# jasonyaw/CDAE

Hardware: AMD Instinct MI355X
Metric: users/sec (whole node) K=200 ML-10M-shape; Recall@10 parity (higher is better)
Workload: dtype f32

## Files before the change

cdae_amd/csrc/cdae_hip.hip:

```cpp
#include <hip/hip_runtime.h>

#include <cstring>

#include <rocprim/rocprim.hpp>

#include <algorithm>
#include <atomic>
#include <condition_variable>
#include <deque>
#include <mutex>
#include <thread>
#include <chrono>
#include <cmath>
#include <cstdarg>
#include <cstdlib>
#include <cstdio>
#include <cstring>
#include <numeric>
#include <string>
#include <vector>

#include "../../include/cdae_hip.h"
#include "cdae_internal.hpp"
#include "cdae_kernels.hpp"
// ... 61 lines not shown
  uint32_t K = 0, Kp = 0, NI = 1, B = 0;
  uint64_t uid_offset = 0;
  cdae::HyperParams hp{};

  std::vector<int64_t> h_row_ptr;
  int64_t* d_row_ptr = nullptr;
  uint32_t* d_col = nullptr;
  uint32_t* d_item_order = nullptr;
  uint32_t hot_rows = 0;
  uint32_t late_rows = 0;
  float* d_Ghot = nullptr;
  uint32_t* d_hotdup = nullptr;
  uint32_t* d_late_bits = nullptr;
  uint32_t late_words = 0;
  bool fused_decode = false;
  bool fused_possible = false;
  bool allow_fused = true;
  uint32_t* h_err = nullptr;
  int err_slot = -1;
  uint32_t* d_fused_err = nullptr;
  cdae::FusedGeom fused_geo{};
  bool fused_geo_set = false;
  std::vector<float> h_rank_len;
  uint32_t* d_cold_map = nullptr;
  uint32_t num_cus = 256;
  cdae::DecodeLate decode_late() const { return cdae::DecodeLate{d_Ghot, d_hotdup, late_rows}; }
  cdae::LateFinish late_finish() { return cdae::LateFinish{d_Ghot, d_hotdup, d_item_order, d_D0, d_dup_corr, late_rows}; }
  bool full_unfused = false;
  std::vector<uint32_t> h_unit_ptr;
  uint32_t* d_rank_of = nullptr;
  uint32_t* d_unit_user = nullptr;
  uint32_t* d_unit_ptr = nullptr;
  uint32_t unit_cap = 0;
  float* d_Hpart = nullptr;
  uint32_t* d_uptr_tmp = nullptr;

  float* d_shared = nullptr;
  size_t n_shared = 0, n_matrix = 0;
  size_t off[CDAE_P_COUNT] = {0};
  size_t cnt[CDAE_P_COUNT] = {0};
  float* d_Wu = nullptr;
  float* d_Wu_ag = nullptr;
  float* d_Uu = nullptr;
  float* d_Uu_ag = nullptr;
  float* d_Ssum = nullptr;
  float* d_delta_rows = nullptr;

  uint64_t Ecap = 0;
  struct ExBuf {
    uint32_t* item = nullptr; uint64_t* val = nullptr;
    uint32_t* sorted_item = nullptr; uint64_t* sorted_val = nullptr;
    uint32_t* seg = nullptr;
    uint16_t* key16 = nullptr; uint16_t* sorted_key16 = nullptr;
    uint32_t* dup_of_pos = nullptr; uint32_t* dup_of_ex = nullptr;
    uint32_t* dup_count = nullptr;
    uint32_t* item_count = nullptr; uint32_t* prefix = nullptr; uint32_t* rank = nullptr; uint64_t* bucketed = nullptr;
    uint32_t* tile_hist = nullptr; uint32_t* block_total = nullptr;
    uint32_t* wg_state = nullptr;
    uint32_t* cells = nullptr; uint32_t* cell_flag = nullptr;
    uint32_t cell_tag = 0;
    hipEvent_t ready = nullptr, released = nullptr;
  } ex[3];
  static constexpr int NSETS = 3;
  hipStream_t prep2 = nullptr;
  bool prep2_own = false;
  bool prep2_auto = false;
  float* d_D0 = nullptr;
  uint32_t dup_stripes = 1;
  float* d_dup_corr = nullptr; uint32_t dup_cap = 0;
  float* d_HGpart = nullptr;
  uint32_t Bp = 0, Ip = 0;
  __bf16 *d_Zb = nullptr, *d_ZTb = nullptr, *d_Db = nullptr, *d_DTb = nullptr, *d_Gb = nullptr, *d_GTb = nullptr;
  float* d_dD = nullptr;
  uint8_t* d_has_in = nullptr;
  uint32_t* d_iota = nullptr;
  uint32_t* d_bits_train = nullptr;
  size_t bits_stride = 0;
  uint32_t full_slices = 1;
  bool db_valid = false;
  bool db_rows_valid = false;
  uint32_t zb_rows = 0xFFFFFFFFu;
  uint32_t full_one_stream_max = 2048;
  hipStream_t aux = nullptr;
// ... 195 lines not shown
    float t = 0.f;
    HIPCHK(hipEventElapsedTime(&t, s.a, s.b));
    ms[s.family] += t;
    launches[s.family]++;
    h->pool.push_back(s.a); h->pool.push_back(s.b);
  }
  h->spans.clear();
  if (st) {
    st->ms_sample = ms[F_SAMPLE]; st->ms_sort = ms[F_SORT]; st->ms_encode = ms[F_ENCODE];
    st->ms_decode = ms[F_DECODE]; st->ms_hidden = ms[F_HIDDEN]; st->ms_input = ms[F_INPUT];
    st->launches_decode = launches[F_DECODE];
  }
  return 0;
}

template <class F, class... P> int visit_slots(F& f, P*&... p) {
  int rc = 0;
  ((rc = rc ? rc : f((void**)&p)), ...);
  return rc;
}
template <class F> int visit_device_ptrs(cdae_hip* h, F f) {
  for (auto& b : h->ex)
    CHK(visit_slots(f, b.item, b.val, b.sorted_item, b.sorted_val, b.seg, b.dup_of_pos, b.dup_of_ex, b.dup_count, b.key16, b.sorted_key16,
                    b.item_count, b.prefix, b.rank, b.bucketed, b.tile_hist, b.block_total, b.wg_state, b.cells, b.cell_flag));
  return visit_slots(f, h->d_row_ptr, h->d_col, h->d_item_order, h->d_shared, h->d_Wu, h->d_Wu_ag, h->d_D0, h->d_HGpart, h->d_sort_tmp,
                     h->d_unit_ptr, h->d_Hpart, h->d_uptr_tmp, h->d_Zb, h->d_ZTb, h->d_Db, h->d_DTb, h->d_Gb, h->d_GTb, h->d_dD, h->d_has_in,
                     h->d_Z, h->d_Dz, h->d_HG, h->d_G, h->d_touched, h->d_uids, h->d_rec, h->d_base, h->d_delta, h->d_recv, h->d_snap,
                     h->d_dup_corr, h->d_unit_user, h->d_zeval, h->d_bits, h->d_hpart_eval, h->d_iota, h->d_bits_train,
                     h->d_Uu, h->d_Uu_ag, h->d_Ssum, h->d_delta_rows, h->d_score, h->d_Hsum, h->d_hsum_eval, h->d_iota_eval, h->d_rec_score,
                     h->d_gpos, h->d_ub, h->d_ub_ag, h->d_UVpre, h->d_rank_of, h->d_grow_ptr, h->d_gcol, h->d_gunit_ptr, h->d_gunit_user,
                     h->d_test_ptr, h->d_test_col, h->d_topn_pu, h->d_topn_out, h->d_bucket_cut, h->d_range_of,
                     h->d_Ghot, h->d_hotdup, h->d_late_bits, h->d_cold_map,
                     h->d_rows_ptr, h->d_rows_uid, h->d_rows_col, h->d_rows_tptr, h->d_rows_pu, h->d_rows_tcol, h->d_rows_out);
}

void free_all(cdae_hip* h) {
  (void)visit_device_ptrs(h, [](void** p) { if (*p) (void)hipFree(*p); *p = nullptr; return 0; });
  if (h->d_scalar) (void)hipFree(h->d_scalar);
  for (auto& b : h->ex) {
    if (b.ready) (void)hipEventDestroy(b.ready);
    if (b.released) (void)hipEventDestroy(b.released);
  }
  if (h->h_err) { err_slot_release(h->device, h->err_slot); h->h_err = nullptr; h->d_fused_err = nullptr; h->err_slot = -1; }
  if (h->prep) (void)hipStreamDestroy(h->prep);
  if (h->prep2 && h->prep2_own) (void)hipStreamDestroy(h->prep2);
  if (h->aux) (void)hipStreamDestroy(h->aux);
  if (h->ev_fork) (void)hipEventDestroy(h->ev_fork);
// ... 75 lines not shown
                       use_cells ? x.cells : (uint32_t*)nullptr, x.cell_flag, x.cell_tag);
  } else
  hipLaunchKernelGGL(sample_kernel, dim3((n_units + 3) / 4), dim3(256), 0, st, h->hp, h->d_row_ptr, h->d_col,
                     h->d_unit_ptr + bt.s0, n_units, bt.s0, bt.nb, bt.cidx, seed, epoch, x.item, x.val, x.key16,
                     x.seg, h->counting_sort || bucket ? 0u : 4u * I, x.dup_count, x.dup_of_ex, h->d_unit_user,
                     x.wg_state, (const uint32_t*)h->d_gpos, 0u, 0u, 0u,
                     (const uint16_t*)(use_cells ? h->d_range_of : nullptr), (const uint32_t*)h->d_bucket_cut, h->bucket_ranges,
                     use_cells ? x.cells : (uint32_t*)nullptr, x.cell_flag, x.cell_tag);
  CHK(pr.end());
  CHK(pr.begin(h, F_SORT, st, prof_q));
  const dim3 seg_grid((uint32_t)((bt.E + 256 * SEG_PER_THREAD - 1) / (256 * SEG_PER_THREAD)));
  if (bt.E == 0) {
  } else if (h->mf_seq && !h->prep_force_sort) {
  } else if (bucket) {
    if (!h->bucket_attr_set) {
      HIPCHK(hipFuncSetAttribute((const void*)bucket_sort_kernel, hipFuncAttributeMaxDynamicSharedMemorySize, (int)BK_LDS_BYTES));
      h->bucket_attr_set = true;
    }
    hipLaunchKernelGGL(bucket_sort_kernel, dim3(h->bucket_ranges), dim3(BK_THREADS), BK_LDS_BYTES, st, (const uint16_t*)x.key16, (const uint64_t*)x.val,
                       (uint32_t)bt.E, (const uint32_t*)h->d_bucket_cut, x.wg_state, (const uint32_t*)(use_cells ? x.cells : nullptr), n_units,
                       (const uint32_t*)x.cell_flag, x.cell_tag, x.seg, x.seg + I, (const uint32_t*)h->d_rank_of,
                       x.seg + 2 * (size_t)I, x.seg + 3 * (size_t)I, x.sorted_val, x.bucketed, x.dup_count, h->dup_cap, x.dup_of_pos, x.dup_of_ex,
                       h->dup_stripes, h->d_fused_err);
  } else if (h->counting_sort) {
    const uint32_t n_tiles = (uint32_t)((bt.E + TILE_EX - 1) / TILE_EX);
    const size_t tile_lds = (size_t)I * sizeof(uint32_t);
    if (tile_lds + 1024 > 64 * 1024 && !h->tile_attr_set) {
      HIPCHK(hipFuncSetAttribute((const void*)tile_hist_kernel, hipFuncAttributeMaxDynamicSharedMemorySize, (int)tile_lds));
      HIPCHK(hipFuncSetAttribute((const void*)tile_scatter_kernel, hipFuncAttributeMaxDynamicSharedMemorySize, (int)tile_lds + 1024));
      h->tile_attr_set = true;
    }
    hipLaunchKernelGGL(tile_hist_kernel, dim3(n_tiles), dim3(TILE_THREADS), tile_lds / 2 + 4, st, x.item, (uint32_t)bt.E, I, x.tile_hist);
    hipLaunchKernelGGL(item_tile_scan_kernel, dim3((I + 255) / 256), dim3(256), 0, st, x.tile_hist, n_tiles, I, x.item_count, x.rank, x.block_total);
    hipLaunchKernelGGL(tile_scatter_kernel, dim3(n_tiles), dim3(TILE_THREADS), tile_lds + 128 * sizeof(uint32_t), st, x.item, x.val,
                       (uint32_t)bt.E, I, x.tile_hist, x.item_count, x.rank, x.block_total, x.prefix, x.seg, x.seg + I, x.dup_count, x.bucketed,
                       (const uint32_t*)h->d_rank_of, x.seg + 2 * (size_t)I, x.seg + 3 * (size_t)I);
    hipLaunchKernelGGL(segment_sort_kernel, dim3((I + SEGSORT_ITEMS - 1) / SEGSORT_ITEMS), dim3(SEGSORT_THREADS), 0, st, I, x.prefix, x.bucketed,
                       x.sorted_val, x.item_count, x.dup_count, h->dup_cap, x.dup_of_pos, x.dup_of_ex, h->dup_stripes);
  } else if (x.key16) {
    HIPCHK(rocprim::radix_sort_pairs(sort_tmp, h->sort_tmp_bytes, x.key16, x.sorted_key16, x.val, x.sorted_val,
                                     (size_t)bt.E, 0u, (unsigned)h->sort_bits, st));
    hipLaunchKernelGGL(segment_kernel<uint16_t>, seg_grid, dim3(256), 0, st, x.sorted_key16, x.sorted_val, (uint32_t)bt.E,
                       x.seg, x.seg + I, x.dup_count, h->dup_cap, x.dup_of_pos, x.dup_of_ex, h->dup_stripes,
                       (const uint32_t*)h->d_rank_of, x.seg + 2 * (size_t)I, x.seg + 3 * (size_t)I, shs ? I : 0xFFFFFFFFu);
  } else {
    HIPCHK(rocprim::radix_sort_pairs(sort_tmp, h->sort_tmp_bytes, x.item, x.sorted_item, x.val, x.sorted_val,
                                     (size_t)bt.E, 0u, (unsigned)h->sort_bits, st));
    hipLaunchKernelGGL(segment_kernel<uint32_t>, seg_grid, dim3(256), 0, st, x.sorted_item, x.sorted_val, (uint32_t)bt.E,
                       x.seg, x.seg + I, x.dup_count, h->dup_cap, x.dup_of_pos, x.dup_of_ex, h->dup_stripes,
                       (const uint32_t*)h->d_rank_of, x.seg + 2 * (size_t)I, x.seg + 3 * (size_t)I, shs ? I : 0xFFFFFFFFu);
  }
  CHK(pr.end());
  if (h->cfg.full_output && h->d_bits_train) {
    const uint32_t words = (I + 31) / 32;
    uint32_t* bits = h->d_bits_train + (size_t)b * h->bits_stride;
    hipLaunchKernelGGL(rated_bits_kernel, dim3((bt.nb + 3) / 4), dim3(256), 0, st, h->d_row_ptr, h->d_col, bt.s0, bt.nb, words, bits);
  }
  HIPCHK(hipEventRecord(x.ready, st));
  HIPCHK(hipGetLastError());
  return 0;
}

int fused_geometry(cdae_hip* h, uint32_t hot, uint32_t I) {
  using namespace cdae;
  FusedGeom g{};
  g.hot_wgs = (hot + 3) / 4;
  const uint32_t n_groups = (I - hot + 3) / 4, S = h->num_cus;
  std::vector<float> len(n_groups, 0.f);
  for (uint32_t q = 0; q < n_groups; ++q)
    for (uint32_t j = 0; j < 4 && hot + 4 * q + j < I; ++j) len[q] = std::max(len[q], h->h_rank_len[hot + 4 * q + j]);
  std::vector<uint32_t> by_len(n_groups);
  std::iota(by_len.begin(), by_len.end(), 0u);
  std::stable_sort(by_len.begin(), by_len.end(), [&](uint32_t a, uint32_t b2) { return len[a] > len[b2]; });
  const uint32_t cu0 = std::min(g.hot_wgs, S > 8 ? S - 8 : 0u);
  const uint32_t n_bins = (S - cu0) * 4;
  std::vector<std::vector<uint32_t>> bin(n_bins);
  {
    using Ent = std::pair<float, uint32_t>;
    std::vector<Ent> heap;
    for (uint32_t i = 0; i < n_bins; ++i) heap.push_back({0.f, i});
    auto cmp = [](const Ent& a, const Ent& b2) { return a.first > b2.first || (a.first == b2.first && a.second > b2.second); };
    std::make_heap(heap.begin(), heap.end(), cmp);
    for (uint32_t k = 0; k < n_groups; ++k) {
      const uint32_t q = by_len[k];
      std::pop_heap(heap.begin(), heap.end(), cmp);
      Ent e = heap.back();
      bin[e.second].push_back(q);
      e.first += 4.f + len[q];
      heap.back() = e;
      std::push_heap(heap.begin(), heap.end(), cmp);
    }
  }
  size_t rounds_cold = 0;
  for (auto& v : bin) rounds_cold = std::max(rounds_cold, v.size());
  g.decode_wgs = (uint32_t)std::max<size_t>(rounds_cold, 1) * S;
  std::vector<uint32_t> map((size_t)g.decode_wgs * 4, 0xFFFFFFFFu);
  for (uint32_t i = 0; i < n_bins; ++i) {
    const uint32_t cu = cu0 + i / 4, w = i % 4;
    for (size_t k = 0; k < bin[i].size(); ++k) map[((size_t)k * S + cu) * 4 + w] = bin[i][k];
  }
  if (h->d_cold_map) { HIPCHK(hipFree(h->d_cold_map)); h->d_cold_map = nullptr; }
  CHK(dev_alloc(&h->d_cold_map, map.size()));
  HIPCHK(hipMemcpy(h->d_cold_map, map.data(), map.size() * sizeof(uint32_t), hipMemcpyHostToDevice));
  g.cold_map = h->d_cold_map;
  h->fused_geo = g;
  h->fused_geo_set = true;
  return 0;
}

int launch_decode(cdae_hip* h, cdae_hip::ExBuf& x, const cdae::GatherArgs* fused = nullptr) {
  using namespace cdae;
  hipStream_t st = h->stream;
  const uint32_t I = (uint32_t)h->I;
  const dim3 blk(256);
  const dim3 grid_rows((I + 3) / 4);
#define DECODE_TAIL h->d_item_order, x.seg + 2 * (size_t)I, x.seg + 3 * (size_t)I, x.sorted_val, h->d_Z, h->dec(), h->dec_ag(), \
                    h->P(CDAE_P_BP), h->P(CDAE_P_BP_AG), h->d_HG, h->d_G, h->d_D0, h->d_touched, x.dup_of_pos, h->d_dup_corr
#define DECODE_ARGS h->hp, DECODE_TAIL
#define DECODE_LA(NI_, L_, A_)                                                                                       \
  do {                                                                                                               \
    if (pad) hipLaunchKernelGGL((decode_rows_kernel<NI_, L_, A_, true>), grid_rows, blk, 0, st, DECODE_ARGS);        \
    else hipLaunchKernelGGL((decode_rows_kernel<NI_, L_, A_, false>), grid_rows, blk, 0, st, DECODE_ARGS);           \
  } while (0)
#define DECODE_NI(NI_)                                          \
  do {                                                          \
    if (ce && ada) DECODE_LA(NI_, 5, true);                     \
    else if (ce) DECODE_LA(NI_, 5, false);                      \
    else if (ada) DECODE_LA(NI_, 0, true);                      \
    else DECODE_LA(NI_, 0, false);                              \
  } while (0)
#define DECODE_HY(NV_, NT_)                                                                                           \
  do {                                                                                                                \
    if (fused) {                                                                                                       \
      if (ce && ada) hipLaunchKernelGGL((decode_gather_kernel<NV_, NT_, 5, true>), grid_fu, blk, 0, st, h->hp, hot, geo, late, *fused, DECODE_TAIL);   \
      else if (ce) hipLaunchKernelGGL((decode_gather_kernel<NV_, NT_, 5, false>), grid_fu, blk, 0, st, h->hp, hot, geo, late, *fused, DECODE_TAIL);    \
      else if (ada) hipLaunchKernelGGL((decode_gather_kernel<NV_, NT_, 0, true>), grid_fu, blk, 0, st, h->hp, hot, geo, late, *fused, DECODE_TAIL);    \
      else hipLaunchKernelGGL((decode_gather_kernel<NV_, NT_, 0, false>), grid_fu, blk, 0, st, h->hp, hot, geo, late, *fused, DECODE_TAIL);            \
    }                                                                                                                  \
    else if (ce && ada) hipLaunchKernelGGL((decode_hybrid_kernel<NV_, NT_, 5, true>), grid_hy, blk, 0, st, h->hp, hot, late, DECODE_TAIL);   \
    else if (ce) hipLaunchKernelGGL((decode_hybrid_kernel<NV_, NT_, 5, false>), grid_hy, blk, 0, st, h->hp, hot, late, DECODE_TAIL);    \
    else if (ada) hipLaunchKernelGGL((decode_hybrid_kernel<NV_, NT_, 0, true>), grid_hy, blk, 0, st, h->hp, hot, late, DECODE_TAIL);    \
    else hipLaunchKernelGGL((decode_hybrid_kernel<NV_, NT_, 0, false>), grid_hy, blk, 0, st, h->hp, hot, late, DECODE_TAIL);            \
  } while (0)
#define DECODE_HY_NT(NV_)                                                                        \
  do {                                                                                           \
    if (nt == 1) DECODE_HY(NV_, 1); else if (nt == 2) DECODE_HY(NV_, 2); else DECODE_HY(NV_, 4); \
  } while (0)
  {
    const bool ce = h->cfg.loss_type == CDAE_LOSS_CROSS_ENTROPY, ada = h->cfg.using_adagrad != 0, pad = h->K < h->Kp;
    const uint32_t K = h->K;
    if (K <= 256) {
      const uint32_t hot = std::min<uint32_t>(h->hot_rows, I);
      const uint32_t waves = hot + (I - hot + 3) / 4;
      const dim3 grid_hy((waves + 3) / 4);
      const DecodeLate late = h->decode_late();
      if (fused && !h->fused_geo_set) CHK(fused_geometry(h, hot, I));
      const FusedGeom geo = h->fused_geo;
      const dim3 grid_fu(geo.decode_wgs + (fused ? 8u * ((fused->n_units + 3u) / 4u) : 0u));
      const uint32_t nv = K / 64, tail = K % 64;
      const uint32_t nt = tail == 0 ? 0u : (tail < 16 ? 1u : (tail < 32 ? 2u : 4u));
      if (nt == 0) {
        switch (nv) { case 1: DECODE_HY(1, 0); break; case 2: DECODE_HY(2, 0); break; case 3: DECODE_HY(3, 0); break; default: DECODE_HY(4, 0); break; }
      } else {
        switch (nv) { case 0: DECODE_HY_NT(0); break; case 1: DECODE_HY_NT(1); break; case 2: DECODE_HY_NT(2); break; default: DECODE_HY_NT(3); break; }
      }
    } else {
      switch (h->NI) { case 1: DECODE_NI(1); break; case 2: DECODE_NI(2); break; case 4: DECODE_NI(4); break; default: DECODE_NI(8); break; }
    }
  }
#undef DECODE_HY_NT
#undef DECODE_HY
#undef DECODE_LA
#undef DECODE_NI
#undef DECODE_ARGS
#undef DECODE_TAIL
  HIPCHK(hipGetLastError());
  return 0;
}
// ... 37 lines not shown
  float* const ghot = h->late_rows ? h->d_Ghot : nullptr;
  uint32_t* const gfill = fused ? reinterpret_cast<uint32_t*>(h->d_G) : nullptr;
  const uint32_t n_fill = fused ? (uint32_t)bt.E : 0u;
  if (!explicit_in && !h->encode_two_launches && nb <= ENCODE_USERS_MAX) {
    DISPATCH_NI(h->NI, encode_users_kernel, dim3(nb), dim3(ENC_WAVES * WAVE), 0, st, h->hp, h->d_row_ptr, h->d_col, h->P(CDAE_P_W), uptr, s0, nb,
                bt.cidx, seed, epoch, h->d_Wu, h->P(CDAE_P_B), h->d_Z, h->d_Dz, h->d_HG, h->d_Uu, h->d_Ssum,
                (BF16_T*)nullptr, (BF16_T*)nullptr, 0u, (float*)nullptr, (const float*)nullptr, (const float*)nullptr, (const uint32_t*)nullptr,
                ghot, h->d_hotdup, gfill, n_fill);
  } else {
    DISPATCH_NI(h->NI, encode_partial_kernel, grid_units, blk, 0, st, h->hp, h->d_row_ptr, h->d_col, h->P(CDAE_P_W), uptr, n_units,
                (const uint32_t*)nullptr, s0, nb, 1, CDAE_STREAM_CORRUPT, bt.cidx, seed, epoch, h->d_Hpart, explicit_in, n_explicit,
                explicit_in ? (const uint32_t*)nullptr : (const uint32_t*)h->d_unit_user);
    DISPATCH_NI(h->NI, encode_finish_kernel, grid_users, blk, 0, st, h->hp, h->d_Hpart, uptr, h->d_Wu, h->P(CDAE_P_B),
                (const uint32_t*)nullptr, s0, nb, 1, h->d_Z, h->d_Dz, h->d_HG, h->d_Uu, h->d_Ssum,
                (BF16_T*)nullptr, (BF16_T*)nullptr, 0u, ghot, h->d_hotdup, gfill, n_fill);
  }
  CHK(pr.end());

  if (!h->skip_ready_wait) HIPCHK(hipStreamWaitEvent(st, x.ready, 0));
  const GatherArgs ga{h->d_row_ptr, uptr, n_units, s0, nb, x.item, h->d_G, h->d_D0, h->d_HGpart, explicit_in ? (uint32_t)bt.E : 0u, x.dup_of_ex,
                      h->d_dup_corr, explicit_in ? (const uint32_t*)nullptr : (const uint32_t*)h->d_unit_user,
                      h->late_rows ? (const uint32_t*)h->d_late_bits : (const uint32_t*)nullptr, h->late_words, h->d_fused_err};
  CHK(pr.begin(h, F_DECODE, st));
  CHK(launch_decode(h, x, fused ? &ga : nullptr));
  CHK(pr.end());

  CHK(pr.begin(h, F_HIDDEN, st));
  if (!fused)
    DISPATCH_NI(h->NI, hidden_gather_kernel, dim3(8 * ((n_units + 3) / 4)), blk, 0, st, h->hp, ga.row_ptr, uptr, n_units, s0, nb,
                x.item, h->d_G, h->d_D0, h->d_HGpart, ga.explicit_examples, x.dup_of_ex, h->d_dup_corr, ga.unit_user,
                ga.late_bits, ga.late_words);
  return sampled_tail(h, x, s0, nb, uptr, n_units, 8u, nullptr, h->late_finish(), &pr);
}

template <int EPI>
int launch_gemm_lds(cdae_hip* h, hipStream_t st, const __bf16* A, const __bf16* Bm, uint32_t M, uint32_t N, uint32_t Kd, uint32_t lda,
                    uint32_t ldb, uint32_t kps, const cdae::GemmEpilogue& ep, uint32_t splits, uint32_t mode) {
  using namespace cdae;
  const uint32_t Nt = (N + 127) / 128;
  if (M % 256 == 0 && N % 256 == 0 && !h->gemm_narrow) {
    if (!h->gemmw_attr_set[EPI]) {
      HIPCHK(hipFuncSetAttribute((const void*)gemm_nt_bf16_ldsw_kernel<EPI>, hipFuncAttributeMaxDynamicSharedMemorySize, (int)gemmw_lds_bytes()));
      h->gemmw_attr_set[EPI] = true;
    }
    const GemmGrid gg{M / 256, N / 256, splits, mode};
    hipLaunchKernelGGL((gemm_nt_bf16_ldsw_kernel<EPI>), dim3(gg.workgroups()), dim3(512), gemmw_lds_bytes(), st, A, Bm, M, N, Kd, lda, ldb,
                       kps, ep, gg);
// ... 731 lines not shown
      const double per_range = std::max(total / 256.0, std::min(2730.0, total / 8.0));
      std::vector<uint32_t> cut{0u};
      double acc = 0.0;
      for (uint64_t i = 0; i < I; ++i) {
        acc += wgt[i];
        if (i + 1 < I && (acc >= per_range || (i + 1) - cut.back() == cdae::BK_ITEMS)) { cut.push_back((uint32_t)(i + 1)); acc = 0.0; }
      }
      cut.push_back((uint32_t)I);
      if (cut.size() - 1 <= cdae::BK_MAX_RANGES) {
        h->bucket_sort = true;
        h->bucket_ranges = (uint32_t)cut.size() - 1;
        CHK(dev_alloc(&h->d_bucket_cut, cut.size()));
        HIPCHK(hipMemcpy(h->d_bucket_cut, cut.data(), cut.size() * sizeof(uint32_t), hipMemcpyHostToDevice));
        if (!h->mf && h->bucket_ranges <= cdae::BKC_MAX_RANGES && h->Ecap < (1ull << (32 - cdae::BKC_ITEM_BITS)) && !DEV_ENV("CDAE_SORT_SCAN")) {
          std::vector<uint16_t> rof(I);
          for (uint32_t r = 0; r + 1 < cut.size(); ++r)
            for (uint32_t i = cut[r]; i < cut[r + 1]; ++i) rof[i] = (uint16_t)r;
          CHK(dev_alloc(&h->d_range_of, (size_t)I));
          HIPCHK(hipMemcpy(h->d_range_of, rof.data(), I * sizeof(uint16_t), hipMemcpyHostToDevice));
        }
      }
    }
  }
  h->h_unit_ptr.assign(U + 1, 0u);
  for (uint64_t u = 0; u < U; ++u)
    h->h_unit_ptr[u + 1] = h->h_unit_ptr[u] + (uint32_t)((row_ptr[u + 1] - row_ptr[u] + h->hp.unit_pos - 1) / h->hp.unit_pos);
  h->unit_cap = 0;
  for (uint64_t s0 = 0; s0 < U; ++s0) {
    const uint64_t s1 = std::min<uint64_t>(U, s0 + B);
    h->unit_cap = std::max(h->unit_cap, h->h_unit_ptr[s1] - h->h_unit_ptr[s0]);
  }
  {
    std::vector<uint32_t> per(U);
    for (uint64_t u = 0; u < U; ++u) per[u] = h->h_unit_ptr[u + 1] - h->h_unit_ptr[u];
    std::partial_sort(per.begin(), per.begin() + B, per.end(), std::greater<uint32_t>());
    uint64_t top = 0;
    for (uint32_t i = 0; i < B; ++i) top += per[i];
    h->unit_cap = (uint32_t)std::max<uint64_t>(h->unit_cap, top);
  }
  if (h->shard_sampled())
    for (uint64_t s0 = 0; s0 < U; ++s0)
      h->unit_cap = std::max(h->unit_cap, h->h_gunit_ptr[std::min<uint64_t>(U, s0 + B)] - h->h_gunit_ptr[s0]);
  CHK(dev_alloc(&h->d_unit_ptr, U + 1));
  HIPCHK(hipMemcpy(h->d_unit_ptr, h->h_unit_ptr.data(), (U + 1) * sizeof(uint32_t), hipMemcpyHostToDevice));
  {
    std::vector<uint32_t> unit_user(h->h_unit_ptr[U]);
// ... 13 lines not shown
  if (h->Ecap > 0xFFFFFFF0ull) return fail("batch of %u users holds %llu examples (> 2^32); lower batch_users", B, (unsigned long long)h->Ecap);
  for (auto& b : h->ex) {
    CHK(dev_alloc(&b.item, h->Ecap)); CHK(dev_alloc(&b.val, h->Ecap));
    CHK(dev_alloc(&b.sorted_item, h->Ecap)); CHK(dev_alloc(&b.sorted_val, h->Ecap));
    CHK(dev_alloc(&b.seg, 4 * (size_t)I));
    CHK(dev_alloc(&b.dup_of_pos, h->Ecap)); CHK(dev_alloc(&b.dup_of_ex, h->Ecap)); CHK(dev_alloc(&b.dup_count, cdae::DUP_STRIPES));
    if (h->counting_sort) {
      CHK(dev_alloc(&b.item_count, (size_t)I)); CHK(dev_alloc(&b.prefix, (size_t)I + 1));
      CHK(dev_alloc(&b.rank, (size_t)I)); CHK(dev_alloc(&b.bucketed, h->Ecap));
      CHK(dev_alloc(&b.tile_hist, (size_t)((h->Ecap + cdae::TILE_EX - 1) / cdae::TILE_EX + 1) * I));
      CHK(dev_alloc(&b.block_total, 128));
    } else if (I + (h->shard_sampled() ? 1u : 0u) <= 65536) { CHK(dev_alloc(&b.key16, h->Ecap + 8)); CHK(dev_alloc(&b.sorted_key16, h->Ecap)); }
    if (h->bucket_sort) { CHK(dev_alloc(&b.bucketed, h->Ecap)); }
    b.cell_tag = 0;
    if (h->bucket_sort && h->d_range_of) {
      const size_t words = (size_t)h->bucket_ranges * h->unit_cap * cdae::BKC_SLOTS;
      if (h->unit_cap <= cdae::BK_CELL_UNITS_MAX && words * sizeof(uint32_t) <= (256ull << 20)) {
        CHK(dev_alloc(&b.cells, words));
        CHK(dev_alloc(&b.cell_flag, 1));
        HIPCHK(hipMemset(b.cell_flag, 0, sizeof(uint32_t)));
        h->cell_units = h->unit_cap;
      }
    }
    CHK(dev_alloc(&b.wg_state, cdae::BK_MAX_RANGES));
    HIPCHK(hipMemset(b.wg_state, 0, cdae::BK_MAX_RANGES * sizeof(uint32_t)));
    if (!b.ready) { HIPCHK(hipEventCreateWithFlags(&b.ready, sync_event_flags())); HIPCHK(hipEventCreateWithFlags(&b.released, sync_event_flags())); }
    HIPCHK(hipEventRecord(b.released, h->stream));
  }
  CHK(dev_alloc(&h->d_D0, IK));
  {
    const char* ev = DEV_ENV("CDAE_DUP_CAP");
    const uint64_t want = h->mf ? 1 : (ev ? std::strtoull(ev, nullptr, 10) : std::max<uint64_t>(65536, h->Ecap / 4));
    h->dup_cap = (uint32_t)std::min<uint64_t>(std::max<uint64_t>(want, 1), std::max<uint64_t>(h->Ecap, 1));
    h->dup_stripes = std::max<uint32_t>(1u, std::min<uint32_t>(cdae::DUP_STRIPES, h->dup_cap / 4096u));
    if ((uint64_t)h->dup_cap * h->Kp * 4u >= (1ull << 31)) h->fused_possible = h->fused_decode = false;
    CHK(dev_alloc(&h->d_dup_corr, (size_t)h->dup_cap * h->Kp));
    HIPCHK(hipMemset(h->d_dup_corr, 0, (size_t)h->dup_cap * h->Kp * sizeof(float)));
  }
  CHK(dev_alloc(&h->d_G, h->Ecap));
  if (h->mf) {
    const uint64_t inst_cap = emax * (h->mf == 2 ? h->hp.num_neg : 1u + h->hp.num_neg);
    CHK(dev_alloc(&h->d_UVpre, (size_t)inst_cap * h->Kp));
    CHK(dev_alloc(&h->d_ub, (size_t)U)); CHK(dev_alloc(&h->d_ub_ag, (size_t)U));
    h->cnt[CDAE_P_UB] = h->cnt[CDAE_P_UB_AG] = (size_t)U;
    HIPCHK(hipMemset(h->d_ub, 0, (size_t)U * sizeof(float)));
  }
// ... 1283 lines not shown
  HIPCHK(hipGetLastError());
  return 0;
}

int fs_phase1(cdae_hip_t* h, uint64_t s0, uint32_t nb) {
  using namespace cdae;
  HIPCHK(hipSetDevice(h->device));
  Batch bt;
  CHK(fs_batch(h, s0, nb, 0, &bt));
  const int b = (int)(h->seq & 1);
  cdae_hip::ExBuf& x = h->ex[b];
  hipStream_t st = h->stream;
  const uint32_t I = (uint32_t)h->I, Kp = h->Kp, Bp = h->Bp, Ip = h->Ip;
  const dim3 blk(256), grid_users((nb + 3) / 4);
  const float* wu_b = gathered_wu(h, h->d_Hsum, nb);
  const float* uu_b = gathered_uu(h, h->d_Hsum, nb);
  if (!h->cfg.full_output) {
    DISPATCH_NI(h->NI, encode_finish_kernel, grid_users, blk, 0, st, h->hp, h->d_Hsum, (const uint32_t*)h->d_iota, wu_b, h->P(CDAE_P_B),
                (const uint32_t*)h->d_iota, s0, nb, 1, h->d_Z, h->d_Dz, h->d_HG, uu_b, h->d_Ssum,
                (BF16_T*)nullptr, (BF16_T*)nullptr, 0u, h->late_rows ? h->d_Ghot : (float*)nullptr, h->d_hotdup);
    HIPCHK(hipStreamWaitEvent(st, x.ready, 0));
    Prof pr;
    CHK(pr.begin(h, F_DECODE, st, h->seq));
    CHK(launch_decode(h, x));
    CHK(pr.end());
    const uint32_t n_gunits = gunits_of(h, bt);
    const uint32_t* guptr = h->d_gunit_ptr + s0;
    if (n_gunits)
      DISPATCH_NI(h->NI, hidden_gather_kernel, dim3(8 * ((n_gunits + 3) / 4)), blk, 0, st, h->hp, h->d_grow_ptr, guptr, n_gunits, s0, nb,
                  x.item, h->d_G, h->d_D0, h->d_HGpart, 0u, x.dup_of_ex, h->d_dup_corr, (const uint32_t*)h->d_gunit_user,
                  h->late_rows ? (const uint32_t*)h->d_late_bits : (const uint32_t*)nullptr, h->late_words);
    DISPATCH_NI(h->NI, hg_raw_kernel, dim3(nb), blk, 0, st, h->hp, guptr, n_gunits, nb, h->d_HGpart, 8u, h->d_HG, h->late_finish());
    HIPCHK(hipGetLastError());
    return 0;
  }
  if (!(rows_fused_path(h) && gemm2_tn_path(h) && h->db_rows_valid))
    hipLaunchKernelGGL(to_bf16_transpose_kernel, dim3(Kp / 64, Ip / 64), blk, 0, st, h->dec(), I, Kp, Kp, Ip, h->d_Db, h->d_DTb);
  CHK(join_aux(h));
  DISPATCH_NI(h->NI, encode_finish_kernel, grid_users, blk, 0, st, h->hp, h->d_Hsum, (const uint32_t*)h->d_iota, wu_b, h->P(CDAE_P_B),
              (const uint32_t*)h->d_iota, s0, nb, 1, h->d_Z, h->d_Dz, h->d_HG, uu_b, h->d_Ssum);
  hipLaunchKernelGGL(to_bf16_transpose_kernel, dim3(Kp / 64, Bp / 64), blk, 0, st, h->d_Z, nb, Kp, Kp, Bp, h->d_Zb, h->d_ZTb);
  HIPCHK(hipStreamWaitEvent(st, x.ready, 0));
  uint32_t parts = 0, rows = nb;
  if (Kp <= 256 && !h->full_unfused) {
    CHK(launch_full_fused(h, st, b, nb));
    parts = h->full_slices; rows = nb;
  } else {
// ... 84 lines not shown
```

cdae_amd/csrc/cdae_kernels.hpp:

```cpp
#pragma once
#include <type_traits>

#include <hip/hip_runtime.h>
#include <stdint.h>

#include "../../include/cdae_rng.h"
#include "cdae_exchange_algebra.h"

namespace cdae {

constexpr int WAVE = 64;
constexpr uint32_t SLOT_MASK = 0x0FFFFFFFu;
constexpr uint32_t DUP_PREV_BIT = 1u << 28;
constexpr uint32_t DUP_NEXT_BIT = 1u << 29;
constexpr uint32_t DUP_NONE = 0xFFFFFFFFu;
constexpr uint32_t DUP_STRIPES = 64;
constexpr uint32_t TARGET_BIT = 1u << 30;
constexpr uint32_t INPUT_BIT = 1u << 31;

constexpr uint32_t LATE_MAX = 64;
struct DecodeLate {
  float* Ghot;
  uint32_t* hotdup;
  uint32_t late_rows;
// ... 1035 lines not shown
  }
#pragma unroll
  for (int i = 0; i < NT; ++i) base[64 * NV + l + 16 * i] = r[4 * NV + i];
}

template <int NV, int NT>
__device__ __forceinline__ void row16_store_sc1(float* __restrict__ matrix, uint32_t row_elem, const float (&r)[4 * NV + NT], uint32_t l) {
  const cdae_rsrc rs = rows_rsrc(matrix);
#pragma unroll
  for (int v = 0; v < NV; ++v) {
    cdae_b128 q; const float t[4] = {r[4 * v], r[4 * v + 1], r[4 * v + 2], r[4 * v + 3]};
    __builtin_memcpy(&q, t, sizeof q);
    __builtin_amdgcn_raw_buffer_store_b128(q, rs, (int)((row_elem + 64u * v + 4u * l) * 4u), 0, AUX_SC1);
  }
#pragma unroll
  for (int i = 0; i < NT; ++i)
    __builtin_amdgcn_raw_buffer_store_b32(__builtin_bit_cast(unsigned int, r[4 * NV + i]), rs, (int)((row_elem + 64u * NV + l + 16u * i) * 4u), 0, AUX_SC1);
}

constexpr uint32_t ROWS16_LDS_WORDS = 4u * 128u + 4u * 128u + 4u * 64u;
constexpr uint32_t ROW64_PARK_WORDS = ROWS16_LDS_WORDS;

template <int NV, int NT, int LOSS, bool ADAGRAD, bool FUSED = false>
__device__ __forceinline__ void decode_rows16(HyperParams hp, const uint32_t rank0, uint32_t* __restrict__ lds, CDAE_DECODE_PARAMS) {
  constexpr int GRP = 16, NE = 4 * NV + NT;
  constexpr bool HAS_PAD = NT > 0;
  const uint32_t lane = threadIdx.x % WAVE, l = lane & (GRP - 1), sub = lane / GRP;
  const uint32_t rank = rank0 + sub;
  const bool row_ok = rank < hp.num_items;
  const uint32_t item = row_ok ? item_order[rank] : 0u;
  const uint32_t beg = row_ok ? seg_begin[rank] : 0u, end = row_ok ? seg_end[rank] : 0u;
  const uint32_t n = end - beg;
  const uint32_t nmax = max(max((uint32_t)__builtin_amdgcn_readlane((int)n, 0), (uint32_t)__builtin_amdgcn_readlane((int)n, 16)),
                            max((uint32_t)__builtin_amdgcn_readlane((int)n, 32), (uint32_t)__builtin_amdgcn_readlane((int)n, 48)));
  if (nmax == 0) return;
  hp.loss_type = LOSS;
  hp.adagrad = ADAGRAD;
#ifdef CDAE_DECODE_TIMING
  unsigned long long* dbg = reinterpret_cast<unsigned long long*>(touched);
  int dbg_n = 0;
#define CDAE_STAMP() do { if (rank0 == hp.debug_rank && lane == 0 && dbg_n < 60) dbg[dbg_n++] = __builtin_readcyclecounter(); } while (0)
#else
#define CDAE_STAMP() do {} while (0)
#endif
  CDAE_STAMP();
  const bool tied = !hp.asymmetric;
  const bool pad_lane = HAS_PAD && l == GRP - 1;
  const float pad_one = pad_lane ? 1.f : 0.f;

  float w[NE], a[NE], wref[NE];
  const size_t row_off = (size_t)item * hp.Kp;
  if (n) {
// ... 149 lines not shown
  if (FLUSH == 16u) flush_sixteen((nmax - 1u) & ~15u);
  else flush_chunk((nmax - 1u) & ~63u);
  if (n) {
    if (HAS_PAD) {
      if (pad_lane) { bp[item] = w[NE - 1]; bp_ag[item] = a[NE - 1]; w[NE - 1] = 0.f; a[NE - 1] = 1.f; }
    } else if (l == 0) {
      bp[item] = bias; bp_ag[item] = bias_ag;
    }
    row16_store<NV, NT>(D + row_off, w, l);
    row16_store<NV, NT>(D_ag + row_off, a, l);
#ifndef CDAE_DECODE_TIMING
    if (l == 0 && touched) touched[item] = 1u;
#endif
  }
#ifdef CDAE_DECODE_TIMING
  CDAE_STAMP();
  if (rank0 == hp.debug_rank && lane == 0) dbg[63] = (unsigned long long)dbg_n | ((unsigned long long)nmax << 32);
#endif
#undef CDAE_STAMP
}

template <int NV, int NT, int LOSS, bool ADAGRAD>
__global__ void __launch_bounds__(256)
decode_hybrid_kernel(HyperParams hp, uint32_t hot_rows, DecodeLate late, CDAE_DECODE_PARAMS) {
  constexpr int CH = NT == 0 ? NV : NV + 1;
  constexpr int NI = CH <= 1 ? 1 : (CH <= 2 ? 2 : 4);
  __shared__ uint32_t rows16_lds[4][ROWS16_LDS_WORDS];
  const uint32_t wave = __builtin_amdgcn_readfirstlane(blockIdx.x * (blockDim.x / WAVE) + threadIdx.x / WAVE);
  if (wave < hot_rows) {
    if (CDAE_SKIP_ROLE(hp, 4u)) return;
    const unsigned long long t0 = trace_begin(hp);
#ifndef CDAE_HOT_PRIO
#define CDAE_HOT_PRIO 2
#endif
    __builtin_amdgcn_s_setprio(CDAE_HOT_PRIO);
    decode_row64<NI, LOSS, ADAGRAD, false>(hp, wave, reinterpret_cast<float*>(rows16_lds[threadIdx.x / WAVE]), ROW64_PARK_WORDS, late,
                                           CDAE_DECODE_PASS);
    trace_end(hp, 3, wave, t0);
  } else {
    if (CDAE_SKIP_ROLE(hp, 8u)) return;
    const unsigned long long t0 = trace_begin(hp);
    decode_rows16<NV, NT, LOSS, ADAGRAD>(hp, hot_rows + (wave - hot_rows) * 4u, rows16_lds[threadIdx.x / WAVE], CDAE_DECODE_PASS);
    trace_end(hp, 4, wave, t0);
  }
}

struct GatherArgs {
  const int64_t* row_ptr; const uint32_t* uptr; uint32_t n_units; uint64_t u0; uint32_t nb;
  const uint32_t* ex_item; const float* G; const float* D0; float* HGpart;
  uint32_t explicit_examples;
  const uint32_t* dup_of_ex; const float* dup_corr; const uint32_t* unit_user;
  const uint32_t* late_bits; uint32_t late_words;
  uint32_t* err;
};
constexpr uint32_t GATHER_CAP = 448;
constexpr uint32_t LATE_BITS_WORDS = 2048;

__device__ __forceinline__ void stage_late_bits(uint32_t* lbits, const uint32_t* __restrict__ late_bits, uint32_t late_words) {
  if (late_bits) {
    for (uint32_t i = threadIdx.x; i < late_words; i += blockDim.x) lbits[i] = late_bits[i];
    __syncthreads();
  }
}

template <int NI, bool FUSED>
// ... 128 lines not shown
  __shared__ uint32_t lbits[LATE_BITS_WORDS];
  stage_late_bits(lbits, late_bits, late_words);
  const uint32_t part = blockIdx.x & 7u;
  const uint32_t unit = (blockIdx.x >> 3) * (blockDim.x / WAVE) + threadIdx.x / WAVE;
  if (unit >= n_units) return;
  const GatherArgs ga{row_ptr, uptr, n_units, u0, nb, ex_item, G, D0, HGpart, explicit_examples, dup_of_ex, dup_corr, unit_user,
                      late_bits, late_words, nullptr};
  hidden_gather_role<NI, false>(hp, ga, part, unit, gl_row[threadIdx.x / WAVE], gl_g[threadIdx.x / WAVE], late_bits ? lbits : nullptr);
}

struct FusedGeom {
  uint32_t hot_wgs;
  uint32_t decode_wgs;
  const uint32_t* cold_map;
};
constexpr uint32_t FUSED_LDS_WORDS = 4u * 2u * GATHER_CAP + LATE_BITS_WORDS;
static_assert(4u * ROWS16_LDS_WORDS <= FUSED_LDS_WORDS, "row roles' LDS");
static_assert(3u * (FUSED_LDS_WORDS + 8u) * 4u + 90376u <= 160u * 1024u, "three workgroups of this launch + one of bucket_sort_kernel per CU");
#ifndef CDAE_FUSED_WAVES_PER_SIMD
#define CDAE_FUSED_WAVES_PER_SIMD 3
#endif
template <int NV, int NT, int LOSS, bool ADAGRAD>
__global__ void __launch_bounds__(256, CDAE_FUSED_WAVES_PER_SIMD)
decode_gather_kernel(HyperParams hp, uint32_t hot_rows, FusedGeom geo, DecodeLate late, GatherArgs ga, CDAE_DECODE_PARAMS) {
  constexpr int CH = NT == 0 ? NV : NV + 1;
  constexpr int NI = CH <= 1 ? 1 : (CH <= 2 ? 2 : 4);
  __shared__ uint32_t fused_lds[FUSED_LDS_WORDS + 8u];
  const uint32_t wg = blockIdx.x;
  const uint32_t wid = __builtin_amdgcn_readfirstlane(threadIdx.x / WAVE);
  if (wg < geo.hot_wgs) {
    const uint32_t row = wg * 4u + wid;
    if (row < hot_rows && !CDAE_SKIP_ROLE(hp, 4u)) {
      const unsigned long long t0 = trace_begin(hp);
      __builtin_amdgcn_s_setprio(CDAE_HOT_PRIO);
      decode_row64<NI, LOSS, ADAGRAD, false, true>(hp, row, reinterpret_cast<float*>(fused_lds + wid * ROWS16_LDS_WORDS), ROW64_PARK_WORDS, late,
                                                   CDAE_DECODE_PASS);
      __builtin_amdgcn_s_setprio(0);
      trace_end(hp, 3, row, t0, hp.trace ? hw_place() : 0u);
    }
  } else if (wg < geo.decode_wgs) {
    if (CDAE_SKIP_ROLE(hp, 8u)) return;
    uint32_t* const claim = fused_lds + FUSED_LDS_WORDS;
    if (threadIdx.x < 4) claim[threadIdx.x] = 0u;
    __syncthreads();
    const uint32_t simd = (__builtin_amdgcn_s_getreg((1 << 11) | (4 << 6) | 4) ) & 3u;
    if (threadIdx.x % WAVE == 0) atomicCAS(&claim[simd], 0u, 1u + wid);
    __syncthreads();
    const uint32_t cs[4] = {claim[0], claim[1], claim[2], claim[3]};
    int mine = -1;
#pragma unroll
    for (int q = 0; q < 4; ++q) if (cs[q] == 1u + wid) mine = q;
    if (mine < 0) {
      uint32_t before = 0, cnt = 0;
#pragma unroll
      for (int q = 0; q < 4; ++q) if (cs[q] && cs[q] - 1u < wid) ++before;
      const uint32_t j = wid - before;
#pragma unroll
      for (int q = 0; q < 4; ++q) if (!cs[q]) { if (cnt == j) mine = q; ++cnt; }
    }
    const uint32_t g = geo.cold_map[wg * 4u + (uint32_t)mine];
    if (g == 0xFFFFFFFFu) return;
    const unsigned long long t0 = trace_begin(hp);
    decode_rows16<NV, NT, LOSS, ADAGRAD, true>(hp, hot_rows + g * 4u, fused_lds + wid * ROWS16_LDS_WORDS, CDAE_DECODE_PASS);
    trace_end(hp, 4, hot_rows / 4u + g, t0, hp.trace ? hw_place() : 0u);
  } else {
    uint32_t* const lbits = fused_lds + 4u * 2u * GATHER_CAP;
    stage_late_bits(lbits, ga.late_bits, ga.late_words);
    const uint32_t gw = wg - geo.decode_wgs;
    const uint32_t part = gw & 7u, unit = (gw >> 3) * 4u + wid;
    if (unit >= ga.n_units) return;
    hidden_gather_role<NI, true>(hp, ga, part, unit, fused_lds + wid * 2u * GATHER_CAP,
                                 reinterpret_cast<float*>(fused_lds + wid * 2u * GATHER_CAP + GATHER_CAP), ga.late_bits ? lbits : nullptr);
  }
}

template <int NI>
__device__ __forceinline__ void add_partial_rows(float (&hg)[NI], const float* __restrict__ HGpart, uint32_t n_units, uint32_t n_parts,
                                                 uint32_t ub, uint32_t ue, uint32_t Kp, uint32_t lo) {
  if (n_parts == 8u) {
    const size_t slab = (size_t)n_units * Kp;
    for (uint32_t u = ub; u < ue; u += 2) {
      const bool two = u + 1u < ue;
      const float* p0 = HGpart + (size_t)u * Kp + lo;
      const float* p1 = HGpart + (size_t)(two ? u + 1u : u) * Kp + lo;
      float a0[8][NI], a1[8][NI];
#pragma unroll
// ... 703 lines not shown
```

cdae_amd/csrc/cdae_sort_kernels.hpp:

```cpp
#pragma once
#include <hip/hip_runtime.h>
#include <stdint.h>

#include "cdae_kernels.hpp"

namespace cdae {

#ifndef CDAE_SEGSORT_THREADS
#define CDAE_SEGSORT_THREADS 256
#endif
constexpr uint32_t SEGSORT_THREADS = CDAE_SEGSORT_THREADS;
#ifndef CDAE_SEGSORT_ITEMS
#define CDAE_SEGSORT_ITEMS 8
#endif
constexpr uint32_t SEGSORT_ITEMS = CDAE_SEGSORT_ITEMS;
#ifndef CDAE_SEGSORT_WINDOW
#define CDAE_SEGSORT_WINDOW 3072
#endif
constexpr uint32_t SEGSORT_WINDOW = CDAE_SEGSORT_WINDOW;

constexpr uint32_t TILE_SORT_MAX_ITEMS = 32768;
#ifndef CDAE_TILE_EX
#define CDAE_TILE_EX 4096
#endif
// ... 438 lines not shown
      if (flags & DUP_PREV_BIT) ++my_dups;
    }
    uint32_t o = my_dups ? atomicAdd(&misc[17], my_dups) : 0u;
    __syncthreads();
    if (t == 0) { misc[18] = misc[17] ? atomicAdd(dup_count + w % stripes, misc[17]) : 0u; misc[17] = 0u; }
    __syncthreads();
    if (my_dups) {
      o += misc[18];
      const uint32_t stripe_cap = dup_cap / stripes, stripe0 = (w % stripes) * stripe_cap;
      for (uint32_t q = t; q < n; q += BK_THREADS) {
        const uint64_t v = sorted_val[base + g0 + q];
        if (!((uint32_t)v & DUP_PREV_BIT)) continue;
        const uint32_t idx = o < stripe_cap ? stripe0 + o : DUP_NONE;
        ++o;
        dup_of_pos[base + g0 + q] = idx;
        dup_of_ex[(uint32_t)(v >> 32)] = idx;
      }
    }
    __syncthreads();
    ia = ib;
  }
}

}
```

Baseline: 2.901 million.

## Order cold decode rows by actual per-batch segment length for load balance

Adds a single-workgroup kernel after the bucket sort that counting-sorts the cold item rows by their actual per-batch segment length, longest first, into a cold_rank table. The decode kernels then map each 4-row cold group through this table, so rows grouped together have similar lengths and long rows are scheduled first. The host geometry builder estimates group lengths from a Poisson model of the expected row length rather than using per-rank maxima. The cost is an extra tiny kernel launch per batch and an indirection load per row, and it is enabled by default when bucket sort is on.

```diff
diff --git a/cdae_amd/csrc/cdae_hip.hip b/cdae_amd/csrc/cdae_hip.hip
--- a/cdae_amd/csrc/cdae_hip.hip
+++ b/cdae_amd/csrc/cdae_hip.hip
@@ -107,6 +107,7 @@
   cdae::FusedGeom fused_geo{};
   bool fused_geo_set = false;
   std::vector<float> h_rank_len;
+  bool cold_order = false;
   uint32_t* d_cold_map = nullptr;
   uint32_t num_cus = 256;
   cdae::DecodeLate decode_late() const { return cdae::DecodeLate{d_Ghot, d_hotdup, late_rows}; }
@@ -144,6 +145,7 @@
     uint32_t* wg_state = nullptr;
     uint32_t* cells = nullptr; uint32_t* cell_flag = nullptr;
     uint32_t cell_tag = 0;
+    uint32_t* cold_rank = nullptr;
     hipEvent_t ready = nullptr, released = nullptr;
   } ex[3];
   static constexpr int NSETS = 3;
@@ -385,7 +387,7 @@
 template <class F> int visit_device_ptrs(cdae_hip* h, F f) {
   for (auto& b : h->ex)
     CHK(visit_slots(f, b.item, b.val, b.sorted_item, b.sorted_val, b.seg, b.dup_of_pos, b.dup_of_ex, b.dup_count, b.key16, b.sorted_key16,
-                    b.item_count, b.prefix, b.rank, b.bucketed, b.tile_hist, b.block_total, b.wg_state, b.cells, b.cell_flag));
+                    b.item_count, b.prefix, b.rank, b.bucketed, b.tile_hist, b.block_total, b.wg_state, b.cells, b.cell_flag, b.cold_rank));
   return visit_slots(f, h->d_row_ptr, h->d_col, h->d_item_order, h->d_shared, h->d_Wu, h->d_Wu_ag, h->d_D0, h->d_HGpart, h->d_sort_tmp,
                      h->d_unit_ptr, h->d_Hpart, h->d_uptr_tmp, h->d_Zb, h->d_ZTb, h->d_Db, h->d_DTb, h->d_Gb, h->d_GTb, h->d_dD, h->d_has_in,
                      h->d_Z, h->d_Dz, h->d_HG, h->d_G, h->d_touched, h->d_uids, h->d_rec, h->d_base, h->d_delta, h->d_recv, h->d_snap,
@@ -507,6 +509,9 @@
                        (const uint32_t*)x.cell_flag, x.cell_tag, x.seg, x.seg + I, (const uint32_t*)h->d_rank_of,
                        x.seg + 2 * (size_t)I, x.seg + 3 * (size_t)I, x.sorted_val, x.bucketed, x.dup_count, h->dup_cap, x.dup_of_pos, x.dup_of_ex,
                        h->dup_stripes, h->d_fused_err);
+    if (x.cold_rank)
+      hipLaunchKernelGGL(cold_order_kernel, dim3(1), dim3(CO_THREADS), 0, st, (const uint32_t*)(x.seg + 2 * (size_t)I), (const uint32_t*)(x.seg + 3 * (size_t)I),
+                         std::min<uint32_t>(h->hot_rows, I), I, x.cold_rank);
   } else if (h->counting_sort) {
     const uint32_t n_tiles = (uint32_t)((bt.E + TILE_EX - 1) / TILE_EX);
     const size_t tile_lds = (size_t)I * sizeof(uint32_t);
@@ -552,6 +557,24 @@
   g.hot_wgs = (hot + 3) / 4;
   const uint32_t n_groups = (I - hot + 3) / 4, S = h->num_cus;
   std::vector<float> len(n_groups, 0.f);
+  if (h->cold_order) {
+    constexpr uint32_t NB = cdae::CO_BINS;
+    std::vector<double> rows_of(NB, 0.0);
+    for (uint32_t r = hot; r < I; ++r) {
+      const double m = std::max(0.0, (double)h->h_rank_len[r]);
+      if (m > 200.0) { rows_of[std::min<uint32_t>((uint32_t)(m + 0.5), NB - 1)] += 1.0; continue; }
+      double pk = std::exp(-m), tail = 1.0;
+      for (uint32_t k = 0; k + 1 < NB && tail > 1e-9; ++k) { rows_of[k] += pk; tail -= pk; pk *= m / (double)(k + 1); }
+    }
+    double cum = 0.0;
+    size_t p = 0;
+    const size_t n_cold = I - hot;
+    for (uint32_t k = NB; k-- > 1 && p < n_cold;) {
+      cum += rows_of[k];
+      for (const size_t upto = std::min<size_t>(n_cold, (size_t)(cum + 0.5)); p < upto; ++p)
+        if (p % 4 == 0) len[p / 4] = (float)k;
+    }
+  } else
   for (uint32_t q = 0; q < n_groups; ++q)
     for (uint32_t j = 0; j < 4 && hot + 4 * q + j < I; ++j) len[q] = std::max(len[q], h->h_rank_len[hot + 4 * q + j]);
   std::vector<uint32_t> by_len(n_groups);
@@ -593,7 +616,11 @@
   return 0;
 }
 
-int launch_decode(cdae_hip* h, cdae_hip::ExBuf& x, const cdae::GatherArgs* fused = nullptr) {
+inline bool cold_table_valid(const cdae_hip* h, const cdae_hip::ExBuf& x, uint64_t E) {
+  return h->cold_order && x.cold_rank && h->bucket_sort && x.key16 && E > 0;
+}
+
+int launch_decode(cdae_hip* h, cdae_hip::ExBuf& x, bool cold, const cdae::GatherArgs* fused = nullptr) {
   using namespace cdae;
   hipStream_t st = h->stream;
   const uint32_t I = (uint32_t)h->I;
@@ -617,15 +644,15 @@
 #define DECODE_HY(NV_, NT_)                                                                                           \
   do {                                                                                                                \
     if (fused) {                                                                                                       \
-      if (ce && ada) hipLaunchKernelGGL((decode_gather_kernel<NV_, NT_, 5, true>), grid_fu, blk, 0, st, h->hp, hot, geo, late, *fused, DECODE_TAIL);   \
-      else if (ce) hipLaunchKernelGGL((decode_gather_kernel<NV_, NT_, 5, false>), grid_fu, blk, 0, st, h->hp, hot, geo, late, *fused, DECODE_TAIL);    \
-      else if (ada) hipLaunchKernelGGL((decode_gather_kernel<NV_, NT_, 0, true>), grid_fu, blk, 0, st, h->hp, hot, geo, late, *fused, DECODE_TAIL);    \
-      else hipLaunchKernelGGL((decode_gather_kernel<NV_, NT_, 0, false>), grid_fu, blk, 0, st, h->hp, hot, geo, late, *fused, DECODE_TAIL);            \
+      if (ce && ada) hipLaunchKernelGGL((decode_gather_kernel<NV_, NT_, 5, true>), grid_fu, blk, 0, st, h->hp, hot, geo, late, *fused, cold_rank, DECODE_TAIL);   \
+      else if (ce) hipLaunchKernelGGL((decode_gather_kernel<NV_, NT_, 5, false>), grid_fu, blk, 0, st, h->hp, hot, geo, late, *fused, cold_rank, DECODE_TAIL);    \
+      else if (ada) hipLaunchKernelGGL((decode_gather_kernel<NV_, NT_, 0, true>), grid_fu, blk, 0, st, h->hp, hot, geo, late, *fused, cold_rank, DECODE_TAIL);    \
+      else hipLaunchKernelGGL((decode_gather_kernel<NV_, NT_, 0, false>), grid_fu, blk, 0, st, h->hp, hot, geo, late, *fused, cold_rank, DECODE_TAIL);            \
     }                                                                                                                  \
-    else if (ce && ada) hipLaunchKernelGGL((decode_hybrid_kernel<NV_, NT_, 5, true>), grid_hy, blk, 0, st, h->hp, hot, late, DECODE_TAIL);   \
-    else if (ce) hipLaunchKernelGGL((decode_hybrid_kernel<NV_, NT_, 5, false>), grid_hy, blk, 0, st, h->hp, hot, late, DECODE_TAIL);    \
-    else if (ada) hipLaunchKernelGGL((decode_hybrid_kernel<NV_, NT_, 0, true>), grid_hy, blk, 0, st, h->hp, hot, late, DECODE_TAIL);    \
-    else hipLaunchKernelGGL((decode_hybrid_kernel<NV_, NT_, 0, false>), grid_hy, blk, 0, st, h->hp, hot, late, DECODE_TAIL);            \
+    else if (ce && ada) hipLaunchKernelGGL((decode_hybrid_kernel<NV_, NT_, 5, true>), grid_hy, blk, 0, st, h->hp, hot, late, cold_rank, DECODE_TAIL);   \
+    else if (ce) hipLaunchKernelGGL((decode_hybrid_kernel<NV_, NT_, 5, false>), grid_hy, blk, 0, st, h->hp, hot, late, cold_rank, DECODE_TAIL);    \
+    else if (ada) hipLaunchKernelGGL((decode_hybrid_kernel<NV_, NT_, 0, true>), grid_hy, blk, 0, st, h->hp, hot, late, cold_rank, DECODE_TAIL);    \
+    else hipLaunchKernelGGL((decode_hybrid_kernel<NV_, NT_, 0, false>), grid_hy, blk, 0, st, h->hp, hot, late, cold_rank, DECODE_TAIL);            \
   } while (0)
 #define DECODE_HY_NT(NV_)                                                                        \
   do {                                                                                           \
@@ -639,6 +666,7 @@
       const uint32_t waves = hot + (I - hot + 3) / 4;
       const dim3 grid_hy((waves + 3) / 4);
       const DecodeLate late = h->decode_late();
+      const uint32_t* const cold_rank = cold ? x.cold_rank : nullptr;
       if (fused && !h->fused_geo_set) CHK(fused_geometry(h, hot, I));
       const FusedGeom geo = h->fused_geo;
       const dim3 grid_fu(geo.decode_wgs + (fused ? 8u * ((fused->n_units + 3u) / 4u) : 0u));
@@ -722,7 +750,7 @@
                       h->d_dup_corr, explicit_in ? (const uint32_t*)nullptr : (const uint32_t*)h->d_unit_user,
                       h->late_rows ? (const uint32_t*)h->d_late_bits : (const uint32_t*)nullptr, h->late_words, h->d_fused_err};
   CHK(pr.begin(h, F_DECODE, st));
-  CHK(launch_decode(h, x, fused ? &ga : nullptr));
+  CHK(launch_decode(h, x, !explicit_in && cold_table_valid(h, x, bt.E), fused ? &ga : nullptr));
   CHK(pr.end());
 
   CHK(pr.begin(h, F_HIDDEN, st));
@@ -1500,6 +1528,10 @@
       }
     }
   }
+  {
+    const char* ev = DEV_ENV("CDAE_COLD_ORDER");
+    h->cold_order = h->bucket_sort && h->K <= 256 && !h->mf && !h->cfg.full_output && !(ev && std::atoi(ev) == 0);
+  }
   h->h_unit_ptr.assign(U + 1, 0u);
   for (uint64_t u = 0; u < U; ++u)
     h->h_unit_ptr[u + 1] = h->h_unit_ptr[u] + (uint32_t)((row_ptr[u + 1] - row_ptr[u] + h->hp.unit_pos - 1) / h->hp.unit_pos);
@@ -1559,6 +1591,7 @@
         h->cell_units = h->unit_cap;
       }
     }
+    if (h->cold_order) CHK(dev_alloc(&b.cold_rank, (size_t)I));
     CHK(dev_alloc(&b.wg_state, cdae::BK_MAX_RANGES));
     HIPCHK(hipMemset(b.wg_state, 0, cdae::BK_MAX_RANGES * sizeof(uint32_t)));
     if (!b.ready) { HIPCHK(hipEventCreateWithFlags(&b.ready, sync_event_flags())); HIPCHK(hipEventCreateWithFlags(&b.released, sync_event_flags())); }
@@ -2888,7 +2921,7 @@
     HIPCHK(hipStreamWaitEvent(st, x.ready, 0));
     Prof pr;
     CHK(pr.begin(h, F_DECODE, st, h->seq));
-    CHK(launch_decode(h, x));
+    CHK(launch_decode(h, x, cold_table_valid(h, x, bt.E)));
     CHK(pr.end());
     const uint32_t n_gunits = gunits_of(h, bt);
     const uint32_t* guptr = h->d_gunit_ptr + s0;
diff --git a/cdae_amd/csrc/cdae_kernels.hpp b/cdae_amd/csrc/cdae_kernels.hpp
--- a/cdae_amd/csrc/cdae_kernels.hpp
+++ b/cdae_amd/csrc/cdae_kernels.hpp
@@ -1081,12 +1081,16 @@
 constexpr uint32_t ROW64_PARK_WORDS = ROWS16_LDS_WORDS;
 
 template <int NV, int NT, int LOSS, bool ADAGRAD, bool FUSED = false>
-__device__ __forceinline__ void decode_rows16(HyperParams hp, const uint32_t rank0, uint32_t* __restrict__ lds, CDAE_DECODE_PARAMS) {
+__device__ __forceinline__ void decode_rows16(HyperParams hp, const uint32_t hot_rows, const uint32_t group,
+                                              const uint32_t* __restrict__ cold_rank, uint32_t* __restrict__ lds, CDAE_DECODE_PARAMS) {
   constexpr int GRP = 16, NE = 4 * NV + NT;
   constexpr bool HAS_PAD = NT > 0;
   const uint32_t lane = threadIdx.x % WAVE, l = lane & (GRP - 1), sub = lane / GRP;
-  const uint32_t rank = rank0 + sub;
-  const bool row_ok = rank < hp.num_items;
+  const uint32_t pos = 4u * group + sub;
+  [[maybe_unused]] const uint32_t rank0 = hot_rows + 4u * group;
+  const bool pos_ok = hot_rows + pos < hp.num_items;
+  const uint32_t rank = cold_rank ? (pos_ok ? cold_rank[pos] : hp.num_items) : hot_rows + pos;
+  const bool row_ok = pos_ok && rank < hp.num_items;
   const uint32_t item = row_ok ? item_order[rank] : 0u;
   const uint32_t beg = row_ok ? seg_begin[rank] : 0u, end = row_ok ? seg_end[rank] : 0u;
   const uint32_t n = end - beg;
@@ -1282,7 +1286,7 @@
 
 template <int NV, int NT, int LOSS, bool ADAGRAD>
 __global__ void __launch_bounds__(256)
-decode_hybrid_kernel(HyperParams hp, uint32_t hot_rows, DecodeLate late, CDAE_DECODE_PARAMS) {
+decode_hybrid_kernel(HyperParams hp, uint32_t hot_rows, DecodeLate late, const uint32_t* __restrict__ cold_rank , CDAE_DECODE_PARAMS) {
   constexpr int CH = NT == 0 ? NV : NV + 1;
   constexpr int NI = CH <= 1 ? 1 : (CH <= 2 ? 2 : 4);
   __shared__ uint32_t rows16_lds[4][ROWS16_LDS_WORDS];
@@ -1300,7 +1304,7 @@
   } else {
     if (CDAE_SKIP_ROLE(hp, 8u)) return;
     const unsigned long long t0 = trace_begin(hp);
-    decode_rows16<NV, NT, LOSS, ADAGRAD>(hp, hot_rows + (wave - hot_rows) * 4u, rows16_lds[threadIdx.x / WAVE], CDAE_DECODE_PASS);
+    decode_rows16<NV, NT, LOSS, ADAGRAD>(hp, hot_rows, wave - hot_rows, cold_rank, rows16_lds[threadIdx.x / WAVE], CDAE_DECODE_PASS);
     trace_end(hp, 4, wave, t0);
   }
 }
@@ -1475,7 +1479,8 @@
 #endif
 template <int NV, int NT, int LOSS, bool ADAGRAD>
 __global__ void __launch_bounds__(256, CDAE_FUSED_WAVES_PER_SIMD)
-decode_gather_kernel(HyperParams hp, uint32_t hot_rows, FusedGeom geo, DecodeLate late, GatherArgs ga, CDAE_DECODE_PARAMS) {
+decode_gather_kernel(HyperParams hp, uint32_t hot_rows, FusedGeom geo, DecodeLate late, GatherArgs ga, const uint32_t* __restrict__ cold_rank ,
+                     CDAE_DECODE_PARAMS) {
   constexpr int CH = NT == 0 ? NV : NV + 1;
   constexpr int NI = CH <= 1 ? 1 : (CH <= 2 ? 2 : 4);
   __shared__ uint32_t fused_lds[FUSED_LDS_WORDS + 8u];
@@ -1514,7 +1519,7 @@
     const uint32_t g = geo.cold_map[wg * 4u + (uint32_t)mine];
     if (g == 0xFFFFFFFFu) return;
     const unsigned long long t0 = trace_begin(hp);
-    decode_rows16<NV, NT, LOSS, ADAGRAD, true>(hp, hot_rows + g * 4u, fused_lds + wid * ROWS16_LDS_WORDS, CDAE_DECODE_PASS);
+    decode_rows16<NV, NT, LOSS, ADAGRAD, true>(hp, hot_rows, g, cold_rank, fused_lds + wid * ROWS16_LDS_WORDS, CDAE_DECODE_PASS);
     trace_end(hp, 4, hot_rows / 4u + g, t0, hp.trace ? hw_place() : 0u);
   } else {
     uint32_t* const lbits = fused_lds + 4u * 2u * GATHER_CAP;
diff --git a/cdae_amd/csrc/cdae_sort_kernels.hpp b/cdae_amd/csrc/cdae_sort_kernels.hpp
--- a/cdae_amd/csrc/cdae_sort_kernels.hpp
+++ b/cdae_amd/csrc/cdae_sort_kernels.hpp
@@ -484,4 +484,38 @@
   }
 }
 
-}
+constexpr uint32_t CO_THREADS = 1024;
+constexpr uint32_t CO_BINS = 1024;
+static_assert(CO_BINS == CO_THREADS, "one bin per thread in the scan");
+
+__global__ void __launch_bounds__(CO_THREADS)
+cold_order_kernel(const uint32_t* __restrict__ segr_begin, const uint32_t* __restrict__ segr_end ,
+                  uint32_t hot, uint32_t num_items, uint32_t* __restrict__ cold_rank ) {
+#ifdef CDAE_PREP_SETPRIO
+  __builtin_amdgcn_s_setprio(CDAE_PREP_SETPRIO);
+#endif
+  __shared__ uint32_t bin[CO_BINS];
+  __shared__ uint32_t wave_tot[CO_THREADS / WAVE];
+  const uint32_t t = threadIdx.x, lane = t % WAVE, wid = t / WAVE;
+  bin[t] = 0u;
+  __syncthreads();
+  for (uint32_t r = hot + t; r < num_items; r += CO_THREADS) atomicAdd(&bin[min(segr_end[r] - segr_begin[r], CO_BINS - 1u)], 1u);
+  __syncthreads();
+  const uint32_t c = bin[CO_BINS - 1u - t];
+  uint32_t incl = c;
+#pragma unroll
+  for (int off = 1; off < WAVE; off <<= 1) {
+    const uint32_t o = __shfl_up(incl, off, WAVE);
+    if ((int)lane >= off) incl += o;
+  }
+  if (lane == WAVE - 1) wave_tot[wid] = incl;
+  __syncthreads();
+  uint32_t before = 0;
+  for (uint32_t w = 0; w < wid; ++w) before += wave_tot[w];
+  bin[CO_BINS - 1u - t] = before + incl - c;
+  __syncthreads();
+  for (uint32_t r = hot + t; r < num_items; r += CO_THREADS)
+    cold_rank[atomicAdd(&bin[min(segr_end[r] - segr_begin[r], CO_BINS - 1u)], 1u)] = r;
+}
+
+}
```

Result: faster. 2.986 million (median of 6 runs) (+2.9%).
